# violetdenim/c3dgs

Measured on AMD Instinct MI355X. Metric: raster views/sec fwd+bwd @1920x1080, higher is better.
Workload: dtype f32; 1 GPU; BASELINE.json configs[2]: synth-v1 3M Gaussians, SH deg 3, indexed-camera rasterizer (QAT inner loop), mark_visible+fwd+bwd, 1 view/step/GPU; gaussians=3000000, width=1920, height=1080, sh_codebook=304096, gaussian_codebook=754096, parallelism=replicas x1

## Files before the change

### c3dgs_amd/csrc/radix_sort.hip

```cpp
#include "common.hpp"
#include "scan_blocks.hpp"
#include <algorithm>
#include <cstdlib>
#include <type_traits>

namespace c3dgs {

constexpr int OS_RADIX = 256;
#ifndef C3DGS_OS_TILE32
#define C3DGS_OS_TILE32 12288
#endif
#ifndef C3DGS_OS_BLOCK32
#define C3DGS_OS_BLOCK32 512
#endif
constexpr int OS_TILE16 = 8192, OS_BLOCK16 = 1024;
template <class K> struct OsShape {
    static constexpr int TILE = sizeof(K) == 2 ? OS_TILE16 : C3DGS_OS_TILE32;
    static constexpr int BLOCK = sizeof(K) == 2 ? OS_BLOCK16 : C3DGS_OS_BLOCK32;
    static constexpr int IPT = TILE / BLOCK;
};
constexpr uint32_t OS_FLAG_AGG = 1u << 30, OS_FLAG_PRE = 2u << 30, OS_CNT_MASK = (1u << 30) - 1;
constexpr int OS_MAX_PASSES = 4;
#ifndef C3DGS_OS_SPIN_LIMIT
#define C3DGS_OS_SPIN_LIMIT (1u << 22)
#endif
constexpr uint32_t OS_SPIN_LIMIT = C3DGS_OS_SPIN_LIMIT;
__device__ uint32_t g_os_error;
#ifdef C3DGS_DIAG
__device__ unsigned long long g_os_times[64 * 8];
#endif
#ifdef C3DGS_OS_TIMING
#define OS_T(slot) if (tid == 0 && (bid & 3) == 0 && (bid >> 2) < 64) g_os_times[(bid >> 2) * 8 + (slot)] = __builtin_readcyclecounter();
#define OS_T_DRAIN() asm volatile("s_waitcnt vmcnt(0)");
#define OS_T_LOADS_DONE()                                                                                    \
    if (key[0] == (K)0x12345678 && val[OS_IPT - 1] == 0x87654321u) kout[0] = key[OS_IPT - 1];                \
    OS_T_DRAIN()
#else
#define OS_T(slot)
#define OS_T_DRAIN()
#define OS_T_LOADS_DONE()
#endif

struct OsPlan { int passes; int bits[OS_MAX_PASSES]; };

constexpr int OS_RADIX3 = 512, OS_BITS3 = 9, OS_BITS3_TOP = 32 - 3 * OS_BITS3;
static_assert(OS_RADIX3 == C3DGS_OS_BLOCK32, "one thread per digit in the biased depth sort's passes");
static_assert(OS_RADIX3 == (1 << DEPTH_SORT3_BITS) && 3 * OS_BITS3 == 27 && DEPTH_KEY_LIMIT3 == DEPTH_KEY_BIAS + (1u << 27) - 1u, "common.hpp's plan");
template <bool XF> __device__ __forceinline__ uint32_t os_digit_src(uint32_t k) { return XF ? depth_key_biased(k) : k; }

static OsPlan os_plan(int total_bits)
{
    OsPlan p;
    p.passes = (total_bits + 7) / 8;
    if (p.passes < 1) p.passes = 1;
    int left = total_bits < 1 ? 1 : total_bits;
    for (int i = 0; i < p.passes; i++) {
        const int b = (left + (p.passes - i) - 1) / (p.passes - i);
        p.bits[i] = b;
        left -= b;
    }
    return p;
}

template <class K> static size_t os_blocks(size_t n) { return (n + OsShape<K>::TILE - 1) / OsShape<K>::TILE; }
template <class K> constexpr bool os_table_driven() { return sizeof(K) == 2; }
template <class K> static size_t os_table_words(size_t n) { return os_table_driven<K>() ? os_blocks<K>(n) * OS_RADIX : 0; }
template <class K> static size_t os_lookback_words(size_t n, int passes)
{
    return os_table_driven<K>() ? 0 : (size_t)passes * os_blocks<K>(n) * OS_RADIX + 64;
}
template <class K> static size_t os_ctrl_bytes(size_t n, int passes)
{
    return align_up(((size_t)passes * OS_RADIX + os_lookback_words<K>(n, passes) + os_table_words<K>(n)) * sizeof(uint32_t));
}

constexpr int OS_HIST_BLOCK = 1024;
template <class K>
__device__ __forceinline__ void os_hist_body(const K* __restrict__ keys, size_t n, const OsPlan& plan, uint32_t* __restrict__ hist,
                                             unsigned block, unsigned nblocks)
{
    __shared__ uint32_t s_h[OS_MAX_PASSES][OS_RADIX];
    for (int q = threadIdx.x; q < OS_MAX_PASSES * OS_RADIX; q += OS_HIST_BLOCK) (&s_h[0][0])[q] = 0;
    __syncthreads();
    constexpr int VEC = 16 / sizeof(K);
    const size_t nvec = n / VEC;
    const uint4* k4 = reinterpret_cast<const uint4*>(keys);
    auto add = [&](uint32_t k) {
        int shift = 0;
        for (int p = 0; p < plan.passes; p++) {
            atomicAdd(&s_h[p][(k >> shift) & ((1u << plan.bits[p]) - 1u)], 1u);
            shift += plan.bits[p];
        }
    };
    auto add4 = [&](const uint4 v) {
        const uint32_t w[4] = { v.x, v.y, v.z, v.w };
#pragma unroll
        for (int e = 0; e < 4; e++) {
            if (sizeof(K) == 4) add(w[e]);
            else { add(w[e] & 0xffffu); add(w[e] >> 16); }
        }
    };
    const size_t stride = (size_t)nblocks * OS_HIST_BLOCK;
    size_t i = (size_t)block * OS_HIST_BLOCK + threadIdx.x;
    for (; i + 3 * stride < nvec; i += 4 * stride) {
        const uint4 v0 = k4[i], v1 = k4[i + stride], v2 = k4[i + 2 * stride], v3 = k4[i + 3 * stride];
        add4(v0); add4(v1); add4(v2); add4(v3);
    }
    for (; i < nvec; i += stride) add4(k4[i]);
    for (size_t j = nvec * VEC + (size_t)block * OS_HIST_BLOCK + threadIdx.x; j < n; j += stride) add((uint32_t)keys[j]);
    __syncthreads();
    for (int q = threadIdx.x; q < plan.passes * OS_RADIX; q += OS_HIST_BLOCK) {
        const uint32_t v = (&s_h[0][0])[q];
        if (v) atomicAdd(&hist[q], v);
    }
}

template <class K>
__global__ void __launch_bounds__(OS_HIST_BLOCK) os_hist_kernel(const K* __restrict__ keys, size_t n, OsPlan plan, uint32_t* __restrict__ hist)
{
    os_hist_body<K>(keys, n, plan, hist, blockIdx.x, gridDim.x);
}

static_assert(SCAN_BLOCKS_THREADS == OS_HIST_BLOCK, "one workgroup shape for both bodies");
__global__ void __launch_bounds__(OS_HIST_BLOCK)
os_hist_scan_kernel(const uint32_t* __restrict__ keys, size_t n, OsPlan plan, uint32_t* __restrict__ hist, int nb, uint32_t* __restrict__ base,
                    const uint32_t* __restrict__ sort_err, uint32_t* __restrict__ host_out, uint32_t host_seq)
{
    if (blockIdx.x == 0) scan_blocks_body(nb, base, sort_err, host_out, host_seq);
    else os_hist_body<uint32_t>(keys, n, plan, hist, blockIdx.x - 1, gridDim.x - 1);
}

__device__ __forceinline__ void os_hist3_body(const uint32_t* __restrict__ keys, size_t n, uint32_t* __restrict__ hist, uint32_t* __restrict__ maxw,
                                              uint32_t* __restrict__ done, uint32_t* __restrict__ host_max, uint32_t host_seq,
                                              unsigned block, unsigned nblocks)
{
    __shared__ uint32_t s_h[3][OS_RADIX3];
    __shared__ uint32_t s_max;
    for (int q = threadIdx.x; q < 3 * OS_RADIX3; q += OS_HIST_BLOCK) (&s_h[0][0])[q] = 0;
    if (threadIdx.x == 0) s_max = 0;
    __syncthreads();
    uint32_t mx = 0;
    auto add = [&](uint32_t k) {
        const uint32_t t = depth_key_biased(k);
        atomicAdd(&s_h[0][t & (OS_RADIX3 - 1)], 1u);
        atomicAdd(&s_h[1][(t >> OS_BITS3) & (OS_RADIX3 - 1)], 1u);
        atomicAdd(&s_h[2][(t >> (2 * OS_BITS3)) & (OS_RADIX3 - 1)], 1u);
        if (k != DEPTH_KEY_CULLED) mx = max(mx, k);
    };
    auto add4 = [&](const uint4 v) { add(v.x); add(v.y); add(v.z); add(v.w); };
    const size_t nvec = n / 4;
    const uint4* k4 = reinterpret_cast<const uint4*>(keys);
    const size_t stride = (size_t)nblocks * OS_HIST_BLOCK;
    size_t i = (size_t)block * OS_HIST_BLOCK + threadIdx.x;
    for (; i + 3 * stride < nvec; i += 4 * stride) {
        const uint4 v0 = k4[i], v1 = k4[i + stride], v2 = k4[i + 2 * stride], v3 = k4[i + 3 * stride];
        add4(v0); add4(v1); add4(v2); add4(v3);
    }
    for (; i < nvec; i += stride) add4(k4[i]);
    for (size_t j = nvec * 4 + (size_t)block * OS_HIST_BLOCK + threadIdx.x; j < n; j += stride) add(keys[j]);
#pragma unroll
    for (int o = 32; o > 0; o >>= 1) mx = max(mx, (uint32_t)__shfl_xor((int)mx, o));
    if ((threadIdx.x & 63) == 0 && mx) atomicMax(&s_max, mx);
    __syncthreads();
    for (int q = threadIdx.x; q < 3 * OS_RADIX3; q += OS_HIST_BLOCK) {
        const uint32_t v = (&s_h[0][0])[q];
        if (v) atomicAdd(&hist[q], v);
    }
    if (threadIdx.x == 0) {
        if (s_max) __hip_atomic_fetch_max(maxw, s_max, __ATOMIC_RELAXED, __HIP_MEMORY_SCOPE_AGENT);
        const uint32_t before = __hip_atomic_fetch_add(done, 1u, __ATOMIC_ACQ_REL, __HIP_MEMORY_SCOPE_AGENT);
        if (before == nblocks - 1 && host_max) {
            const uint32_t m = __hip_atomic_load(maxw, __ATOMIC_RELAXED, __HIP_MEMORY_SCOPE_AGENT);
            __hip_atomic_store(host_max, m, __ATOMIC_RELAXED, __HIP_MEMORY_SCOPE_SYSTEM);
            __hip_atomic_store(host_max + 1, host_seq, __ATOMIC_RELEASE, __HIP_MEMORY_SCOPE_SYSTEM);
        }
    }
}

__global__ void __launch_bounds__(OS_HIST_BLOCK)
os_hist3_scan_kernel(const uint32_t* __restrict__ keys, size_t n, uint32_t* __restrict__ hist, uint32_t* __restrict__ maxw, uint32_t* __restrict__ done,
                     uint32_t* __restrict__ host_max, int nb, uint32_t* __restrict__ base, const uint32_t* __restrict__ sort_err,
                     uint32_t* __restrict__ host_out, uint32_t host_seq)
{
    if (blockIdx.x == 0) scan_blocks_body(nb, base, sort_err, host_out, host_seq);
    else os_hist3_body(keys, n, hist, maxw, done, host_max, host_seq, blockIdx.x - 1, gridDim.x - 1);
}

__global__ void __launch_bounds__(OS_HIST_BLOCK) os_hist3_top_kernel(const uint32_t* __restrict__ keys, size_t n, uint32_t* __restrict__ hist)
{
    __shared__ uint32_t s_h[1 << OS_BITS3_TOP];
    if (threadIdx.x < (1 << OS_BITS3_TOP)) s_h[threadIdx.x] = 0;
    __syncthreads();
    const size_t stride = (size_t)gridDim.x * OS_HIST_BLOCK;
    const size_t rounds = (n + stride - 1) / stride;
    for (size_t r = 0; r < rounds; r++) {
        const size_t i = r * stride + (size_t)blockIdx.x * OS_HIST_BLOCK + threadIdx.x;
        const bool ok = i < n;
        const uint32_t d = ok ? depth_key_biased(keys[i]) >> (3 * OS_BITS3) : 0u;
        unsigned long long left = __ballot(ok);
        while (left) {
            const int leader = __ffsll((long long)left) - 1;
            const uint32_t dl = (uint32_t)__shfl((int)d, leader);
            const unsigned long long same = __ballot(ok && d == dl) & left;
            if ((int)(threadIdx.x & 63) == leader) atomicAdd(&s_h[dl], (uint32_t)__popcll(same));
            left &= ~same;
        }
    }
    __syncthreads();
    if (threadIdx.x < (1 << OS_BITS3_TOP) && s_h[threadIdx.x]) atomicAdd(&hist[threadIdx.x], s_h[threadIdx.x]);
}

__global__ void __launch_bounds__(1024) os_tile_hist_kernel(const uint16_t* __restrict__ keys, uint32_t n, int shift, int bits, uint32_t* __restrict__ table)
{
    constexpr int TILE = OsShape<uint16_t>::TILE;
    static_assert(TILE == 8 * 1024, "one 16-byte load of 8 keys per thread");
    __shared__ uint32_t s_h[OS_RADIX];
    if (threadIdx.x < OS_RADIX) s_h[threadIdx.x] = 0;
    __syncthreads();
    const uint32_t base = blockIdx.x * (uint32_t)TILE + threadIdx.x * 8u;
    const uint32_t mask = (1u << bits) - 1u;
    auto add = [&](uint32_t k) { atomicAdd(&s_h[(k >> shift) & mask], 1u); };
    if (base + 8 <= n && (reinterpret_cast<uintptr_t>(keys) & 15u) == 0) {
        const uint4 v = *reinterpret_cast<const uint4*>(keys + base);
        const uint32_t w[4] = { v.x, v.y, v.z, v.w };
#pragma unroll
        for (int e = 0; e < 4; e++) { add(w[e] & 0xffffu); add(w[e] >> 16); }
    } else {
        for (uint32_t i = base; i < min(base + 8u, n); i++) add((uint32_t)keys[i]);
    }
    __syncthreads();
    const int t = threadIdx.x;
    if (t < (1 << bits)) table[(size_t)t * gridDim.x + blockIdx.x] = s_h[t];
}

constexpr int OS_SCAN_V = 8;
__global__ void __launch_bounds__(256) os_table_scan_kernel(uint32_t* __restrict__ table, uint32_t blocks, uint32_t* __restrict__ hist)
{
    static_assert(OS_RADIX == 256, "one thread per histogram word");
    __shared__ uint32_t s_w[4];
    const int digit = (int)blockIdx.x;
    uint32_t* column = table + (size_t)digit * blocks;
    const int lane = threadIdx.x & 63, wave = threadIdx.x >> 6;
    if (digit == 0 && threadIdx.x >= gridDim.x) hist[threadIdx.x] = 0u;
    uint32_t carry = 0;
    for (uint32_t b0 = 0; b0 < blocks; b0 += 256 * OS_SCAN_V) {
        const uint32_t b = b0 + threadIdx.x * OS_SCAN_V;
        uint32_t c[OS_SCAN_V], mine = 0;
#pragma unroll
        for (int q = 0; q < OS_SCAN_V; q++) { c[q] = b + q < blocks ? column[b + q] : 0u; mine += c[q]; }
        uint32_t incl = mine;
#pragma unroll
        for (int o = 1; o < 64; o <<= 1) { const uint32_t t = __shfl_up(incl, o); if (lane >= o) incl += t; }
        __syncthreads();
        if (lane == 63) s_w[wave] = incl;
        __syncthreads();
        uint32_t run = carry + incl - mine;
        for (int w = 0; w < wave; w++) run += s_w[w];
#pragma unroll
        for (int q = 0; q < OS_SCAN_V; q++) { if (b + q < blocks) column[b + q] = run; run += c[q]; }
        carry += s_w[0] + s_w[1] + s_w[2] + s_w[3];
    }
    if (threadIdx.x == 0) hist[digit] = carry;
}

__device__ __forceinline__ uint32_t os_load(const uint32_t* p) { return __hip_atomic_load(p, __ATOMIC_RELAXED, __HIP_MEMORY_SCOPE_AGENT); }
__device__ __forceinline__ void os_store(uint32_t* p, uint32_t v) { __hip_atomic_store(p, v, __ATOMIC_RELAXED, __HIP_MEMORY_SCOPE_AGENT); }

__device__ __forceinline__ uint32_t os_pack_rect(uint2 r)
{
    return (r.x & 0xffu) | ((r.x >> 16) << 8) | ((r.y & 0xffu) << 16) | ((r.y >> 16) << 24);
}
__device__ __forceinline__ uint2 os_unpack_rect(uint32_t w)
{
    return make_uint2((w & 0xffu) | (((w >> 8) & 0xffu) << 16), ((w >> 16) & 0xffu) | ((w >> 24) << 16));
}

template <class K, int BITS, bool PRE, bool PAY2 = false, int RADIX = OS_RADIX, bool XF = false>
__global__ void __launch_bounds__(OsShape<K>::BLOCK)
os_pass_kernel(const K* __restrict__ kin, K* __restrict__ kout, const uint32_t* __restrict__ vin, uint32_t* __restrict__ vout,
               uint32_t n, int shift, const uint32_t* __restrict__ hist, uint32_t* __restrict__ status, uint32_t* __restrict__ ticket,
               const uint2* __restrict__ gather_src, uint2* __restrict__ gather_dst, const uint32_t* __restrict__ p2in = nullptr,
               uint32_t* __restrict__ p2out = nullptr)
{
    constexpr uint32_t ERR_BIT = sizeof(K) == 2 ? 1u : 2u;
    constexpr uint32_t MASK = (1u << BITS) - 1;
    constexpr int OS_BLOCK = OsShape<K>::BLOCK, OS_IPT = OsShape<K>::IPT, OS_WAVES = OS_BLOCK / 64;
    constexpr int OS_TILE = OsShape<K>::TILE;
    using CNT = typename std::conditional<(RADIX > 256), uint16_t, uint32_t>::type;
    static_assert(RADIX % 64 == 0 && RADIX <= OS_BLOCK && BITS <= 9 && (1 << BITS) <= RADIX, "one thread per digit");
    static_assert(!XF || sizeof(K) == 4, "the transform is the depth keys'");
    static_assert(sizeof(CNT) == 4 || OS_TILE < 65536, "a 16-bit counter holds up to a tile's items");
    static_assert(sizeof(CNT) * OS_WAVES * RADIX + 8 * RADIX + 4 * (RADIX / 64) + 4 + sizeof(K) * OS_TILE + 4 * OS_TILE * (PAY2 ? 2 : 1) + (PAY2 ? 0 : 4)
                      <= 160 * 1024, "LDS of one workgroup (160 KB per CU)");
    __shared__ CNT s_cnt[OS_WAVES][RADIX];
    __shared__ uint32_t s_start[RADIX];
    __shared__ int32_t s_gbase[RADIX];
    __shared__ uint32_t s_wtot[RADIX / 64];
    __shared__ uint32_t s_bid;
    __shared__ K s_keys[OS_TILE];
    __shared__ uint32_t s_vals[OS_TILE];
    __shared__ uint32_t s_vals2[PAY2 ? OS_TILE : 1];

    const int tid = threadIdx.x, lane = tid & 63, wave = tid >> 6;
    if (tid == 0) s_bid = PRE ? blockIdx.x : atomicAdd(ticket, 1u);
    for (int q = tid; q < OS_WAVES * RADIX; q += OS_BLOCK) (&s_cnt[0][0])[q] = 0;
    __syncthreads();
    const uint32_t bid = s_bid;
    OS_T(0)
    const uint32_t block_start = bid * (uint32_t)OS_TILE;
    const uint32_t valid = min((uint32_t)OS_TILE, n - block_start);

    K key[OS_IPT];
    uint32_t val[OS_IPT], rank[OS_IPT];
    uint32_t val2[PAY2 ? OS_IPT : 1];
    const uint32_t wbase = block_start + (uint32_t)wave * 64u * OS_IPT;
#pragma unroll
    for (int k = 0; k < OS_IPT; k++) {
        const uint32_t idx = wbase + (uint32_t)k * 64u + lane;
        const bool ok = idx < n;
        key[k] = ok ? kin[idx] : (K)0;
        val[k] = ok ? (vin ? vin[idx] : idx) : 0u;
        if (PAY2) val2[k] = ok ? (p2in ? p2in[idx] : os_pack_rect(gather_src[idx])) : 0u;
    }
    const uint32_t lt_lo = lane < 32 ? (1u << lane) - 1u : 0xffffffffu, lt_hi = lane < 32 ? 0u : (1u << (lane - 32)) - 1u;
    OS_T_LOADS_DONE()
    OS_T(1)
    CNT* wc = s_cnt[wave];
#pragma unroll
    for (int k = 0; k < OS_IPT; k++) {
        const uint32_t idx = wbase + (uint32_t)k * 64u + lane;
        const bool ok = idx < n;
        const uint32_t d = (os_digit_src<XF>((uint32_t)key[k]) >> shift) & MASK;
        const unsigned long long okb = __ballot(ok);
        uint32_t plo = (uint32_t)okb, phi = (uint32_t)(okb >> 32);
#pragma unroll
        for (int b = 0; b < BITS; b++) {
            const int sgn = __builtin_amdgcn_sbfe((int)d, b, 1);
            const unsigned long long bal = __ballot(sgn != 0);
            plo &= ~((uint32_t)bal ^ (uint32_t)sgn);
            phi &= ~((uint32_t)(bal >> 32) ^ (uint32_t)sgn);
        }
        rank[k] = 0;
        if (ok) {
            const uint32_t before = __hip_atomic_load(&wc[d], __ATOMIC_RELAXED, __HIP_MEMORY_SCOPE_WAVEFRONT);
            const uint32_t below = (uint32_t)__popc(plo & lt_lo) + (uint32_t)__popc(phi & lt_hi);
            rank[k] = before + below;
            if (below == 0) __hip_atomic_store(&wc[d], (CNT)(before + (uint32_t)__popc(plo) + (uint32_t)__popc(phi)), __ATOMIC_RELAXED, __HIP_MEMORY_SCOPE_WAVEFRONT);
        }
        __builtin_amdgcn_fence(__ATOMIC_RELEASE, "wavefront");
        __builtin_amdgcn_wave_barrier();
        __builtin_amdgcn_fence(__ATOMIC_ACQUIRE, "wavefront");
    }
    OS_T(2)
    __syncthreads();
    OS_T(3)
    uint32_t tot = 0;
    if (tid < RADIX) {
#pragma unroll
        for (int w = 0; w < OS_WAVES; w++) { const uint32_t c = s_cnt[w][tid]; s_cnt[w][tid] = (CNT)tot; tot += c; }
    }
    uint32_t incl = tot;
#pragma unroll
    for (int o = 1; o < 64; o <<= 1) { const uint32_t t = __shfl_up(incl, o); if (lane >= o) incl += t; }
    if (tid < RADIX && lane == 63) s_wtot[wave] = incl;
    __syncthreads();
    uint32_t start = 0, pre = 0;
    if (tid < RADIX) {
        uint32_t off = 0;
        for (int w = 0; w < wave; w++) off += s_wtot[w];
        start = off + incl - tot;
        s_start[tid] = start;
        uint32_t* my = status + (size_t)bid * RADIX + tid;
        if (PRE) pre = tid < (1 << BITS) ? status[(size_t)tid * gridDim.x + bid] : 0u;
        else if (bid == 0) os_store(my, OS_FLAG_PRE | tot);
        else {
            os_store(my, OS_FLAG_AGG | tot);
            for (int64_t b = (int64_t)bid - 1;; b--) {
                uint32_t s, spins = 0;
                do { s = os_load(status + (size_t)b * RADIX + tid); } while ((s >> 30) == 0 && ++spins < OS_SPIN_LIMIT);
                if ((s >> 30) == 0) { atomicOr(&g_os_error, ERR_BIT); break; }
                pre += s & OS_CNT_MASK;
                if (s & OS_FLAG_PRE) break;
            }
            os_store(my, OS_FLAG_PRE | (pre + tot));
        }
    }
    OS_T(4)
    const uint32_t h = tid < RADIX ? hist[tid] : 0u;
    uint32_t hincl = h;
#pragma unroll
    for (int o = 1; o < 64; o <<= 1) { const uint32_t t = __shfl_up(hincl, o); if (lane >= o) hincl += t; }
    __syncthreads();
    if (tid < RADIX && lane == 63) s_wtot[wave] = hincl;
    __syncthreads();
    if (tid < RADIX) {
        uint32_t off = 0;
        for (int w = 0; w < wave; w++) off += s_wtot[w];
        s_gbase[tid] = (int32_t)(off + hincl - h + pre) - (int32_t)start;
    }
    OS_T(5)
#pragma unroll
    for (int k = 0; k < OS_IPT; k++) {
        const uint32_t idx = wbase + (uint32_t)k * 64u + lane;
        if (idx < n) {
            const uint32_t d = (os_digit_src<XF>((uint32_t)key[k]) >> shift) & MASK;
            const uint32_t p = s_start[d] + s_cnt[wave][d] + rank[k];
            s_keys[p] = key[k];
            s_vals[p] = val[k];
            if (PAY2) s_vals2[p] = val2[k];
        }
    }
    __syncthreads();
    OS_T(6)
#pragma unroll
    for (int m = 0; m < OS_IPT; m++) {
        const uint32_t p = (uint32_t)tid + (uint32_t)m * OS_BLOCK;
        if (p < valid) {
            const K kk = s_keys[p];
            const uint32_t d = (os_digit_src<XF>((uint32_t)kk) >> shift) & MASK;
            const uint32_t g = (uint32_t)(s_gbase[d] + (int32_t)p);
            kout[g] = kk;
            const uint32_t vv = s_vals[p];
            vout[g] = vv;
            if (PAY2) {
                if (p2out) p2out[g] = s_vals2[p];
                else gather_dst[g] = os_unpack_rect(s_vals2[p]);
            } else if (gather_src) gather_dst[g] = gather_src[vv];
        }
    }
    OS_T_DRAIN()
    OS_T(7)
}

template <class K, bool PRE>
static void os_launch_pass(int bits, unsigned blocks, hipStream_t s, const K* ki, K* ko, const uint32_t* vi, uint32_t* vo, uint32_t n,
                           int shift, const uint32_t* hist, uint32_t* status, uint32_t* ticket, const uint2* gsrc, uint2* gdst)
{
#define C3DGS_OS_CASE(B) case B: os_pass_kernel<K, B, PRE><<<blocks, OsShape<K>::BLOCK, 0, s>>>(ki, ko, vi, vo, n, shift, hist, status, ticket, gsrc, gdst); break
    switch (bits) {
        C3DGS_OS_CASE(1); C3DGS_OS_CASE(2); C3DGS_OS_CASE(3); C3DGS_OS_CASE(4);
        C3DGS_OS_CASE(5); C3DGS_OS_CASE(6); C3DGS_OS_CASE(7);
        default: os_pass_kernel<K, 8, PRE><<<blocks, OsShape<K>::BLOCK, 0, s>>>(ki, ko, vi, vo, n, shift, hist, status, ticket, gsrc, gdst); break;
    }
#undef C3DGS_OS_CASE
}

template <class K> static unsigned os_hist_blocks(size_t n)
{
    const size_t nvec16 = n * sizeof(K) / 16 + 1;
    return (unsigned)std::min<size_t>((nvec16 + OS_HIST_BLOCK * 4 - 1) / (OS_HIST_BLOCK * 4), 512);
}

template <class K>
static size_t os_temp_bytes(size_t n, int total_bits, bool pay2 = false)
{
    const OsPlan plan = os_plan(total_bits);
    size_t b = os_ctrl_bytes<K>(n, plan.passes);
    const int bufs = plan.passes >= 3 ? 2 : (plan.passes == 2 ? 1 : 0);
    b += (size_t)bufs * (align_up(n * sizeof(K)) + align_up(n * sizeof(uint32_t)));
    if (pay2) b += 2 * align_up(n * sizeof(uint32_t));
    return b;
}

template <class K>
static size_t os_clear_bytes(size_t n, int total_bits)
{
    if (os_table_driven<K>()) return 0;
    return os_ctrl_bytes<K>(n, os_plan(total_bits).passes);
}

template <class K>
static hipError_t os_sort(void* temp, size_t temp_bytes, const K* kin, K* kout, const uint32_t* vin, uint32_t* vout, size_t n,
                          int total_bits, hipStream_t s, const uint2* gather_src = nullptr, uint2* gather_dst = nullptr,
                          bool ctrl_cleared = false, bool pay2 = false, bool hist_done = false)
{
    if (n == 0) return hipSuccess;
    if (pay2 && (sizeof(K) != 4 || total_bits != 32 || !gather_src || !gather_dst || vin || os_temp_bytes<K>(n, total_bits, true) > temp_bytes))
        pay2 = false;
    if (n >= ((size_t)1 << 30) || total_bits > 8 * (int)sizeof(K) || os_temp_bytes<K>(n, total_bits) > temp_bytes) return hipErrorInvalidValue;
    const OsPlan plan = os_plan(total_bits);
    const size_t blocks = os_blocks<K>(n);
    char* base = (char*)temp;
    const size_t ctrl = os_ctrl_bytes<K>(n, plan.passes);
    uint32_t* hist = (uint32_t*)base;
    uint32_t* behind_hist = hist + (size_t)plan.passes * OS_RADIX;
    K* tk[2]; uint32_t* tv[2];
    char* q = base + ctrl;
    for (int i = 0; i < 2; i++) { tk[i] = (K*)q; q += align_up(n * sizeof(K)); tv[i] = (uint32_t*)q; q += align_up(n * sizeof(uint32_t)); }
    if constexpr (os_table_driven<K>()) {
        uint32_t* table = behind_hist;
        int shift = 0;
        for (int p = 0; p < plan.passes; p++) {
            const bool last = p == plan.passes - 1;
            const K* ki = p == 0 ? kin : tk[(p - 1) & 1];
            const uint32_t* vi = p == 0 ? vin : tv[(p - 1) & 1];
            uint32_t* h = hist + (size_t)p * OS_RADIX;
            os_tile_hist_kernel<<<(unsigned)blocks, 1024, 0, s>>>((const uint16_t*)ki, (uint32_t)n, shift, plan.bits[p], table);
            os_table_scan_kernel<<<1u << plan.bits[p], 256, 0, s>>>(table, (uint32_t)blocks, h);
            os_launch_pass<K, true>(plan.bits[p], (unsigned)blocks, s, ki, last ? kout : tk[p & 1], vi, last ? vout : tv[p & 1], (uint32_t)n,
                                    shift, h, table, nullptr, last ? gather_src : nullptr, last ? gather_dst : nullptr);
            shift += plan.bits[p];
        }
        return hipGetLastError();
    } else {
        uint32_t* status = behind_hist;
        uint32_t* ticket = status + (size_t)plan.passes * blocks * OS_RADIX;
        uint32_t* t2[2] = { nullptr, nullptr };
        if (pay2) {
            q = base + os_temp_bytes<K>(n, total_bits);
            for (int i = 0; i < 2; i++) { t2[i] = (uint32_t*)q; q += align_up(n * sizeof(uint32_t)); }
        }
        if (!ctrl_cleared) {
            const hipError_t e = hipMemsetAsync(base, 0, os_clear_bytes<K>(n, total_bits), s);
            if (e != hipSuccess) return e;
        }
        if (!hist_done) os_hist_kernel<K><<<os_hist_blocks<K>(n), OS_HIST_BLOCK, 0, s>>>(kin, n, plan, hist);
        int shift = 0;
        for (int p = 0; p < plan.passes; p++) {
            const K* ki = p == 0 ? kin : tk[(p - 1) & 1];
            const uint32_t* vi = p == 0 ? vin : tv[(p - 1) & 1];
            K* ko = p == plan.passes - 1 ? kout : tk[p & 1];
            uint32_t* vo = p == plan.passes - 1 ? vout : tv[p & 1];
            const bool last = p == plan.passes - 1;
            if (pay2)
                os_pass_kernel<K, 8, false, true><<<(unsigned)blocks, OsShape<K>::BLOCK, 0, s>>>(
                    ki, ko, vi, vo, (uint32_t)n, shift, hist + (size_t)p * OS_RADIX, status + (size_t)p * blocks * OS_RADIX, ticket + p,
                    gather_src, gather_dst, p == 0 ? nullptr : t2[(p - 1) & 1], last ? nullptr : t2[p & 1]);
            else
                os_launch_pass<K, false>(plan.bits[p], (unsigned)blocks, s, ki, ko, vi, vo, (uint32_t)n, shift, hist + (size_t)p * OS_RADIX,
                                         status + (size_t)p * blocks * OS_RADIX, ticket + p, last ? gather_src : nullptr, last ? gather_dst : nullptr);
            shift += plan.bits[p];
        }
        return hipGetLastError();
    }
}

struct Os3Layout {
    size_t blocks, ctrl_bytes, total_bytes;
    uint32_t *hist[4], *status[4], *ticket, *maxw, *done;
    uint32_t *tk[2], *tv[2], *t2[2];
};
static Os3Layout os3_layout(void* temp, size_t n)
{
    Os3Layout L;
    L.blocks = os_blocks<uint32_t>(n);
    const size_t hist_words = 3 * OS_RADIX3 + OS_RADIX, status_words = L.blocks * hist_words;
    L.ctrl_bytes = align_up((hist_words + status_words + 64) * sizeof(uint32_t));
    uint32_t* w = (uint32_t*)temp;
    for (int p = 0; p < 4; p++) {
        L.hist[p] = w + (size_t)p * OS_RADIX3;
        L.status[p] = w + hist_words + (size_t)p * L.blocks * OS_RADIX3;
    }
    L.ticket = w + hist_words + status_words;
    L.maxw = L.ticket + 8;
    L.done = L.ticket + 9;
    char* q = (char*)temp + L.ctrl_bytes;
    const size_t a = align_up(n * sizeof(uint32_t));
    for (int i = 0; i < 2; i++) { L.tk[i] = (uint32_t*)q; q += a; L.tv[i] = (uint32_t*)q; q += a; }
    for (int i = 0; i < 2; i++) { L.t2[i] = (uint32_t*)q; q += a; }
    L.total_bytes = (size_t)(q - (char*)temp);
    return L;
}
static bool os3_args_ok(size_t temp_bytes, int P)
{
    return P > 0 && (size_t)P < ((size_t)1 << 30) && os3_layout(nullptr, (size_t)P).total_bytes <= temp_bytes;
}

hipError_t onesweep_depth3_hist_scan(void* temp, size_t temp_bytes, const uint32_t* keys, int P, int nb, uint32_t* base,
                                     const uint32_t* sort_err, uint32_t* host_out, uint32_t host_seq, uint32_t* host_max, hipStream_t s)
{
    if (!os3_args_ok(temp_bytes, P)) return hipErrorInvalidValue;
    const Os3Layout L = os3_layout(temp, (size_t)P);
    os_hist3_scan_kernel<<<1u + os_hist_blocks<uint32_t>((size_t)P), OS_HIST_BLOCK, 0, s>>>(keys, (size_t)P, L.hist[0], L.maxw, L.done, host_max, nb,
                                                                                            base, sort_err, host_out, host_seq);
    return hipGetLastError();
}
const uint32_t* onesweep_depth3_max_word(void* temp, int P) { return os3_layout(temp, (size_t)(P > 0 ? P : 1)).maxw; }

hipError_t onesweep_depth3_head(void* temp, size_t temp_bytes, const uint32_t* kin, int P, const uint2* rects, hipStream_t s)
{
    if (!os3_args_ok(temp_bytes, P) || !rects) return hipErrorInvalidValue;
    const Os3Layout L = os3_layout(temp, (size_t)P);
    const unsigned blocks = (unsigned)L.blocks;
    os_pass_kernel<uint32_t, OS_BITS3, false, true, OS_RADIX3, true><<<blocks, C3DGS_OS_BLOCK32, 0, s>>>(
        kin, L.tk[0], nullptr, L.tv[0], (uint32_t)P, 0, L.hist[0], L.status[0], L.ticket + 0, rects, nullptr, nullptr, L.t2[0]);
    os_pass_kernel<uint32_t, OS_BITS3, false, true, OS_RADIX3, true><<<blocks, C3DGS_OS_BLOCK32, 0, s>>>(
        L.tk[0], L.tk[1], L.tv[0], L.tv[1], (uint32_t)P, OS_BITS3, L.hist[1], L.status[1], L.ticket + 1, rects, nullptr, L.t2[0], L.t2[1]);
    return hipGetLastError();
}
hipError_t onesweep_depth3_tail(void* temp, size_t temp_bytes, const uint32_t* kin, uint32_t* kout, uint32_t* vout, int P,
                                const uint2* rects, uint2* rects_sorted, uint32_t max_visible_key, hipStream_t s)
{
    if (!os3_args_ok(temp_bytes, P) || !rects || !rects_sorted) return hipErrorInvalidValue;
    const Os3Layout L = os3_layout(temp, (size_t)P);
    const unsigned blocks = (unsigned)L.blocks;
    const bool four = depth_sort_plan(true, max_visible_key).passes == 4;
    os_pass_kernel<uint32_t, OS_BITS3, false, true, OS_RADIX3, true><<<blocks, C3DGS_OS_BLOCK32, 0, s>>>(
        L.tk[1], four ? L.tk[0] : kout, L.tv[1], four ? L.tv[0] : vout, (uint32_t)P, 2 * OS_BITS3, L.hist[2], L.status[2], L.ticket + 2, rects,
        rects_sorted, L.t2[1], four ? L.t2[0] : nullptr);
    if (four) {
        os_hist3_top_kernel<<<os_hist_blocks<uint32_t>((size_t)P), OS_HIST_BLOCK, 0, s>>>(kin, (size_t)P, L.hist[3]);
        os_pass_kernel<uint32_t, OS_BITS3_TOP, false, true, OS_RADIX, true><<<blocks, C3DGS_OS_BLOCK32, 0, s>>>(
            L.tk[0], kout, L.tv[0], vout, (uint32_t)P, 3 * OS_BITS3, L.hist[3], L.status[3], L.ticket + 3, rects, rects_sorted, L.t2[0], nullptr);
    }
    return hipGetLastError();
}

#ifdef C3DGS_DIAG
int os_read_times(unsigned long long* out512)
{
    return hipMemcpyFromSymbol(out512, HIP_SYMBOL(g_os_times), sizeof(unsigned long long) * 512) != hipSuccess;
}
#endif

uint32_t* onesweep_error_word()
{
    static uint32_t* cache[64] = { nullptr };
    int dev = 0;
    if (hipGetDevice(&dev) != hipSuccess || dev < 0 || dev >= 64) return nullptr;
    if (!cache[dev]) {
        void* p = nullptr;
        if (hipGetSymbolAddress(&p, HIP_SYMBOL(g_os_error)) != hipSuccess) return nullptr;
        cache[dev] = (uint32_t*)p;
    }
    return cache[dev];
}

int onesweep_timed_out(hipStream_t s)
{
    if (!onesweep_enabled()) return 0;
    uint32_t* e = onesweep_error_word();
    uint32_t w = 1;
    if (!e || hipMemcpyAsync(&w, e, sizeof(w), hipMemcpyDeviceToHost, s) != hipSuccess) return 1;
    if (hipStreamSynchronize(s) != hipSuccess) return 1;
    if (w) (void)hipMemsetAsync(e, 0, sizeof(w), s);
    return w != 0;
}

bool onesweep_enabled()
{
    static const bool on = []() { const char* e = std::getenv("C3DGS_SORT_ROCPRIM"); return !(e && e[0] == '1'); }();
    return on;
}
size_t onesweep_depth_temp_bytes(int P)
{
    const size_t n = (size_t)(P > 0 ? P : 1);
    return std::max(os_temp_bytes<uint32_t>(n, 32, true), os3_layout(nullptr, n).total_bytes);
}
size_t onesweep_tile_temp_bytes(int R, int end_bit, int key_bytes)
{
    return key_bytes == 4 ? os_temp_bytes<uint32_t>((size_t)(R > 0 ? R : 1), end_bit) : os_temp_bytes<uint16_t>((size_t)(R > 0 ? R : 1), end_bit);
}
size_t onesweep_depth_clear_bytes(int P)
{
    const size_t n = (size_t)(P > 0 ? P : 1);
    return std::max(os_clear_bytes<uint32_t>(n, 32), os3_layout(nullptr, n).ctrl_bytes);
}
size_t onesweep_tile_clear_bytes(int R, int end_bit, int key_bytes)
{
    return key_bytes == 4 ? os_clear_bytes<uint32_t>((size_t)(R > 0 ? R : 1), end_bit) : os_clear_bytes<uint16_t>((size_t)(R > 0 ? R : 1), end_bit);
}
hipError_t onesweep_tile_sort32(void* temp, size_t temp_bytes, const uint32_t* kin, uint32_t* kout, const uint32_t* vin, uint32_t* vout,
                                int R, int end_bit, hipStream_t s, bool ctrl_cleared)
{
    return os_sort<uint32_t>(temp, temp_bytes, kin, kout, vin, vout, (size_t)R, end_bit, s, nullptr, nullptr, ctrl_cleared);
}
hipError_t onesweep_depth_hist_scan(void* temp, size_t temp_bytes, const uint32_t* keys, int P, int nb, uint32_t* base,
                                    const uint32_t* sort_err, uint32_t* host_out, uint32_t host_seq, hipStream_t s)
{
    const size_t n = (size_t)P;
    if (P <= 0 || n >= ((size_t)1 << 30) || os_temp_bytes<uint32_t>(n, 32) > temp_bytes) return hipErrorInvalidValue;
    os_hist_scan_kernel<<<1u + os_hist_blocks<uint32_t>(n), OS_HIST_BLOCK, 0, s>>>(keys, n, os_plan(32), (uint32_t*)temp, nb, base,
                                                                                  sort_err, host_out, host_seq);
    return hipGetLastError();
}
hipError_t onesweep_depth_sort(void* temp, size_t temp_bytes, const uint32_t* kin, uint32_t* kout, const uint32_t* vin, uint32_t* vout,
                               int P, const uint2* gather_src, uint2* gather_dst, hipStream_t s, bool ctrl_cleared, bool rects_fit_bytes,
                               bool hist_done)
{
    static const bool no_pay2 = []() { const char* e = std::getenv("C3DGS_DEPTH_SORT_GATHER"); return e && e[0] == '1'; }();
    return os_sort<uint32_t>(temp, temp_bytes, kin, kout, vin, vout, (size_t)P, 32, s, gather_src, gather_dst, ctrl_cleared,
                             rects_fit_bytes && !no_pay2, hist_done && ctrl_cleared);
}
hipError_t onesweep_tile_sort(void* temp, size_t temp_bytes, const uint16_t* kin, uint16_t* kout, const uint32_t* vin, uint32_t* vout,
                              int R, int end_bit, hipStream_t s, bool ctrl_cleared)
{
    return os_sort<uint16_t>(temp, temp_bytes, kin, kout, vin, vout, (size_t)R, end_bit, s, nullptr, nullptr, ctrl_cleared);
}

}
```

Before: 646.9 views/s.

## Carry only the high digit byte between u16 radix passes and rebuild keys

In the table-driven 16-bit key sort, the first pass now writes only the upper-digit byte to a uint8 plane instead of full u16 keys. The second pass reads that byte plane and rebuilds the low digit from the bucket start offsets of the first pass (a scan of the first histogram done in the second hist kernel), using a binary search over the bucket starts. This halves intermediate key traffic and temp memory. It adds a binary search per thread plus extra kernel template variants, and the scheme assumes at most two passes.

```diff
diff --git a/c3dgs_amd/csrc/radix_sort.hip b/c3dgs_amd/csrc/radix_sort.hip
--- a/c3dgs_amd/csrc/radix_sort.hip
+++ b/c3dgs_amd/csrc/radix_sort.hip
@@ -65,13 +65,14 @@
 template <class K> static size_t os_blocks(size_t n) { return (n + OsShape<K>::TILE - 1) / OsShape<K>::TILE; }
 template <class K> constexpr bool os_table_driven() { return sizeof(K) == 2; }
 template <class K> static size_t os_table_words(size_t n) { return os_table_driven<K>() ? os_blocks<K>(n) * OS_RADIX : 0; }
+template <class K> constexpr size_t os_lo_words() { return os_table_driven<K>() ? OS_RADIX + 8 : 0; }
 template <class K> static size_t os_lookback_words(size_t n, int passes)
 {
     return os_table_driven<K>() ? 0 : (size_t)passes * os_blocks<K>(n) * OS_RADIX + 64;
 }
 template <class K> static size_t os_ctrl_bytes(size_t n, int passes)
 {
-    return align_up(((size_t)passes * OS_RADIX + os_lookback_words<K>(n, passes) + os_table_words<K>(n)) * sizeof(uint32_t));
+    return align_up(((size_t)passes * OS_RADIX + os_lookback_words<K>(n, passes) + os_lo_words<K>() + os_table_words<K>(n)) * sizeof(uint32_t));
 }
 
 constexpr int OS_HIST_BLOCK = 1024;
@@ -210,10 +211,12 @@
     if (threadIdx.x < (1 << OS_BITS3_TOP) && s_h[threadIdx.x]) atomicAdd(&hist[threadIdx.x], s_h[threadIdx.x]);
 }
 
-__global__ void __launch_bounds__(1024) os_tile_hist_kernel(const uint16_t* __restrict__ keys, uint32_t n, int shift, int bits, uint32_t* __restrict__ table)
+template <class K>
+__global__ void __launch_bounds__(1024) os_tile_hist_kernel(const K* __restrict__ keys, uint32_t n, int shift, int bits, uint32_t* __restrict__ table,
+                                                            const uint32_t* __restrict__ lo_hist = nullptr, uint32_t* __restrict__ lo_start = nullptr)
 {
     constexpr int TILE = OsShape<uint16_t>::TILE;
-    static_assert(TILE == 8 * 1024, "one 16-byte load of 8 keys per thread");
+    static_assert(TILE == 8 * 1024 && (sizeof(K) == 1 || sizeof(K) == 2), "one load of 8 keys per thread: 16 bytes of u16, 8 of u8");
     __shared__ uint32_t s_h[OS_RADIX];
     if (threadIdx.x < OS_RADIX) s_h[threadIdx.x] = 0;
     __syncthreads();
@@ -221,16 +224,41 @@
     const uint32_t mask = (1u << bits) - 1u;
     auto add = [&](uint32_t k) { atomicAdd(&s_h[(k >> shift) & mask], 1u); };
     if (base + 8 <= n && (reinterpret_cast<uintptr_t>(keys) & 15u) == 0) {
-        const uint4 v = *reinterpret_cast<const uint4*>(keys + base);
-        const uint32_t w[4] = { v.x, v.y, v.z, v.w };
-#pragma unroll
-        for (int e = 0; e < 4; e++) { add(w[e] & 0xffffu); add(w[e] >> 16); }
+        if constexpr (sizeof(K) == 2) {
+            const uint4 v = *reinterpret_cast<const uint4*>(keys + base);
+            const uint32_t w[4] = { v.x, v.y, v.z, v.w };
+#pragma unroll
+            for (int e = 0; e < 4; e++) { add(w[e] & 0xffffu); add(w[e] >> 16); }
+        } else {
+            const uint2 v = *reinterpret_cast<const uint2*>(keys + base);
+            const uint32_t w[2] = { v.x, v.y };
+#pragma unroll
+            for (int e = 0; e < 2; e++) { add(w[e] & 0xffu); add((w[e] >> 8) & 0xffu); add((w[e] >> 16) & 0xffu); add(w[e] >> 24); }
+        }
     } else {
         for (uint32_t i = base; i < min(base + 8u, n); i++) add((uint32_t)keys[i]);
     }
     __syncthreads();
     const int t = threadIdx.x;
     if (t < (1 << bits)) table[(size_t)t * gridDim.x + blockIdx.x] = s_h[t];
+    if constexpr (sizeof(K) == 1) {
+        if (blockIdx.x == 0 && lo_start) {
+            __shared__ uint32_t s_w[OS_RADIX / 64];
+            const int lane = t & 63, wave = t >> 6;
+            const uint32_t h = t < OS_RADIX ? lo_hist[t] : 0u;
+            uint32_t incl = h;
+#pragma unroll
+            for (int o = 1; o < 64; o <<= 1) { const uint32_t v = __shfl_up(incl, o); if (lane >= o) incl += v; }
+            if (t < OS_RADIX && lane == 63) s_w[wave] = incl;
+            __syncthreads();
+            if (t < OS_RADIX) {
+                uint32_t off = 0;
+                for (int w = 0; w < wave; w++) off += s_w[w];
+                lo_start[t] = off + incl - h;
+            }
+            if (t == 0) lo_start[OS_RADIX] = n;
+        }
+    }
 }
 
 constexpr int OS_SCAN_V = 8;
@@ -275,13 +303,16 @@
     return make_uint2((w & 0xffu) | (((w >> 8) & 0xffu) << 16), ((w >> 16) & 0xffu) | ((w >> 24) << 16));
 }
 
-template <class K, int BITS, bool PRE, bool PAY2 = false, int RADIX = OS_RADIX, bool XF = false>
+constexpr int OS_PLANE_NONE = 0, OS_PLANE_WRITE = 1, OS_PLANE_READ = 2;
+template <class K, int BITS, bool PRE, bool PAY2 = false, int RADIX = OS_RADIX, bool XF = false, int PLANE = OS_PLANE_NONE>
 __global__ void __launch_bounds__(OsShape<K>::BLOCK)
 os_pass_kernel(const K* __restrict__ kin, K* __restrict__ kout, const uint32_t* __restrict__ vin, uint32_t* __restrict__ vout,
                uint32_t n, int shift, const uint32_t* __restrict__ hist, uint32_t* __restrict__ status, uint32_t* __restrict__ ticket,
                const uint2* __restrict__ gather_src, uint2* __restrict__ gather_dst, const uint32_t* __restrict__ p2in = nullptr,
-               uint32_t* __restrict__ p2out = nullptr)
-{
+               uint32_t* __restrict__ p2out = nullptr, const uint8_t* __restrict__ plane_in = nullptr, uint8_t* __restrict__ plane_out = nullptr,
+               const uint32_t* __restrict__ lo_start = nullptr)
+{
+    static_assert(PLANE == OS_PLANE_NONE || (sizeof(K) == 2 && PRE && !PAY2 && !XF && RADIX == OS_RADIX), "the digit plane is the table-driven u16 sort's");
     constexpr uint32_t ERR_BIT = sizeof(K) == 2 ? 1u : 2u;
     constexpr uint32_t MASK = (1u << BITS) - 1;
     constexpr int OS_BLOCK = OsShape<K>::BLOCK, OS_IPT = OsShape<K>::IPT, OS_WAVES = OS_BLOCK / 64;
@@ -291,7 +322,7 @@
     static_assert(!XF || sizeof(K) == 4, "the transform is the depth keys'");
     static_assert(sizeof(CNT) == 4 || OS_TILE < 65536, "a 16-bit counter holds up to a tile's items");
     static_assert(sizeof(CNT) * OS_WAVES * RADIX + 8 * RADIX + 4 * (RADIX / 64) + 4 + sizeof(K) * OS_TILE + 4 * OS_TILE * (PAY2 ? 2 : 1) + (PAY2 ? 0 : 4)
-                      <= 160 * 1024, "LDS of one workgroup (160 KB per CU)");
+                      + 4 * (PLANE == OS_PLANE_READ ? RADIX + 1 : 1) <= 160 * 1024, "LDS of one workgroup (160 KB per CU)");
     __shared__ CNT s_cnt[OS_WAVES][RADIX];
     __shared__ uint32_t s_start[RADIX];
     __shared__ int32_t s_gbase[RADIX];
@@ -300,10 +331,13 @@
     __shared__ K s_keys[OS_TILE];
     __shared__ uint32_t s_vals[OS_TILE];
     __shared__ uint32_t s_vals2[PAY2 ? OS_TILE : 1];
+    __shared__ uint32_t s_lo[PLANE == OS_PLANE_READ ? RADIX + 1 : 1];
 
     const int tid = threadIdx.x, lane = tid & 63, wave = tid >> 6;
     if (tid == 0) s_bid = PRE ? blockIdx.x : atomicAdd(ticket, 1u);
     for (int q = tid; q < OS_WAVES * RADIX; q += OS_BLOCK) (&s_cnt[0][0])[q] = 0;
+    uint32_t lo_v = 0;
+    if constexpr (PLANE == OS_PLANE_READ) { if (tid <= RADIX) lo_v = lo_start[tid]; }
     __syncthreads();
     const uint32_t bid = s_bid;
     OS_T(0)
@@ -318,7 +352,8 @@
     for (int k = 0; k < OS_IPT; k++) {
         const uint32_t idx = wbase + (uint32_t)k * 64u + lane;
         const bool ok = idx < n;
-        key[k] = ok ? kin[idx] : (K)0;
+        if constexpr (PLANE == OS_PLANE_READ) key[k] = ok ? (K)plane_in[idx] : (K)0;
+        else key[k] = ok ? kin[idx] : (K)0;
         val[k] = ok ? (vin ? vin[idx] : idx) : 0u;
         if (PAY2) val2[k] = ok ? (p2in ? p2in[idx] : os_pack_rect(gather_src[idx])) : 0u;
     }
@@ -330,7 +365,7 @@
     for (int k = 0; k < OS_IPT; k++) {
         const uint32_t idx = wbase + (uint32_t)k * 64u + lane;
         const bool ok = idx < n;
-        const uint32_t d = (os_digit_src<XF>((uint32_t)key[k]) >> shift) & MASK;
+        const uint32_t d = PLANE == OS_PLANE_READ ? (uint32_t)key[k] & MASK : (os_digit_src<XF>((uint32_t)key[k]) >> shift) & MASK;
         const unsigned long long okb = __ballot(ok);
         uint32_t plo = (uint32_t)okb, phi = (uint32_t)(okb >> 32);
 #pragma unroll
@@ -352,8 +387,26 @@
         __builtin_amdgcn_fence(__ATOMIC_ACQUIRE, "wavefront");
     }
     OS_T(2)
+    if constexpr (PLANE == OS_PLANE_READ) { if (tid <= RADIX) s_lo[tid] = lo_v; }
     __syncthreads();
     OS_T(3)
+    if constexpr (PLANE == OS_PLANE_READ) {
+        if (wbase + lane < n) {
+            uint32_t lo_d = 0;
+#pragma unroll
+            for (int step = RADIX / 2; step > 0; step >>= 1)
+                if (s_lo[lo_d + step] <= wbase + lane) lo_d += step;
+            uint32_t lo_next = s_lo[lo_d + 1];
+#pragma unroll
+            for (int k = 0; k < OS_IPT; k++) {
+                const uint32_t idx = wbase + (uint32_t)k * 64u + lane;
+                if (idx < n) {
+                    while (idx >= lo_next) lo_next = s_lo[++lo_d + 1];
+                    key[k] = (K)(((uint32_t)key[k] << shift) | lo_d);
+                }
+            }
+        }
+    }
     uint32_t tot = 0;
     if (tid < RADIX) {
 #pragma unroll
@@ -419,7 +472,8 @@
             const K kk = s_keys[p];
             const uint32_t d = (os_digit_src<XF>((uint32_t)kk) >> shift) & MASK;
             const uint32_t g = (uint32_t)(s_gbase[d] + (int32_t)p);
-            kout[g] = kk;
+            if constexpr (PLANE == OS_PLANE_WRITE) plane_out[g] = (uint8_t)((uint32_t)kk >> (shift + BITS));
+            else kout[g] = kk;
             const uint32_t vv = s_vals[p];
             vout[g] = vv;
             if (PAY2) {
@@ -445,6 +499,23 @@
 #undef C3DGS_OS_CASE
 }
 
+static void os_launch_plane_write(int bits, unsigned blocks, hipStream_t s, const uint16_t* ki, uint8_t* plane, const uint32_t* vi, uint32_t* ids,
+                                  uint32_t n, const uint32_t* hist, uint32_t* table)
+{
+#define C3DGS_OS_CASE(B) case B: os_pass_kernel<uint16_t, B, true, false, OS_RADIX, false, OS_PLANE_WRITE><<<blocks, OS_BLOCK16, 0, s>>>( \
+        ki, nullptr, vi, ids, n, 0, hist, table, nullptr, nullptr, nullptr, nullptr, nullptr, nullptr, plane, nullptr); break
+    switch (bits) { C3DGS_OS_CASE(5); C3DGS_OS_CASE(6); C3DGS_OS_CASE(7); default: C3DGS_OS_CASE(8); }
+#undef C3DGS_OS_CASE
+}
+static void os_launch_plane_read(int bits, unsigned blocks, hipStream_t s, const uint8_t* plane, uint16_t* ko, const uint32_t* ids, uint32_t* vo,
+                                 uint32_t n, int shift, const uint32_t* hist, uint32_t* table, const uint32_t* lo_start)
+{
+#define C3DGS_OS_CASE(B) case B: os_pass_kernel<uint16_t, B, true, false, OS_RADIX, false, OS_PLANE_READ><<<blocks, OS_BLOCK16, 0, s>>>( \
+        nullptr, ko, ids, vo, n, shift, hist, table, nullptr, nullptr, nullptr, nullptr, nullptr, plane, nullptr, lo_start); break
+    switch (bits) { C3DGS_OS_CASE(4); C3DGS_OS_CASE(5); C3DGS_OS_CASE(6); C3DGS_OS_CASE(7); default: C3DGS_OS_CASE(8); }
+#undef C3DGS_OS_CASE
+}
+
 template <class K> static unsigned os_hist_blocks(size_t n)
 {
     const size_t nvec16 = n * sizeof(K) / 16 + 1;
@@ -457,7 +528,8 @@
     const OsPlan plan = os_plan(total_bits);
     size_t b = os_ctrl_bytes<K>(n, plan.passes);
     const int bufs = plan.passes >= 3 ? 2 : (plan.passes == 2 ? 1 : 0);
-    b += (size_t)bufs * (align_up(n * sizeof(K)) + align_up(n * sizeof(uint32_t)));
+    const size_t between = os_table_driven<K>() ? sizeof(uint8_t) : sizeof(K);
+    b += (size_t)bufs * (align_up(n * between) + align_up(n * sizeof(uint32_t)));
     if (pay2) b += 2 * align_up(n * sizeof(uint32_t));
     return b;
 }
@@ -488,19 +560,20 @@
     char* q = base + ctrl;
     for (int i = 0; i < 2; i++) { tk[i] = (K*)q; q += align_up(n * sizeof(K)); tv[i] = (uint32_t*)q; q += align_up(n * sizeof(uint32_t)); }
     if constexpr (os_table_driven<K>()) {
-        uint32_t* table = behind_hist;
-        int shift = 0;
-        for (int p = 0; p < plan.passes; p++) {
-            const bool last = p == plan.passes - 1;
-            const K* ki = p == 0 ? kin : tk[(p - 1) & 1];
-            const uint32_t* vi = p == 0 ? vin : tv[(p - 1) & 1];
-            uint32_t* h = hist + (size_t)p * OS_RADIX;
-            os_tile_hist_kernel<<<(unsigned)blocks, 1024, 0, s>>>((const uint16_t*)ki, (uint32_t)n, shift, plan.bits[p], table);
-            os_table_scan_kernel<<<1u << plan.bits[p], 256, 0, s>>>(table, (uint32_t)blocks, h);
-            os_launch_pass<K, true>(plan.bits[p], (unsigned)blocks, s, ki, last ? kout : tk[p & 1], vi, last ? vout : tv[p & 1], (uint32_t)n,
-                                    shift, h, table, nullptr, last ? gather_src : nullptr, last ? gather_dst : nullptr);
-            shift += plan.bits[p];
-        }
+        uint32_t* lo_start = behind_hist;
+        uint32_t* table = behind_hist + os_lo_words<K>();
+        os_tile_hist_kernel<uint16_t><<<(unsigned)blocks, 1024, 0, s>>>((const uint16_t*)kin, (uint32_t)n, 0, plan.bits[0], table);
+        os_table_scan_kernel<<<1u << plan.bits[0], 256, 0, s>>>(table, (uint32_t)blocks, hist);
+        if (plan.passes == 1) {
+            os_launch_pass<K, true>(plan.bits[0], (unsigned)blocks, s, kin, kout, vin, vout, (uint32_t)n, 0, hist, table, nullptr, gather_src, gather_dst);
+            return hipGetLastError();
+        }
+        uint8_t* plane = (uint8_t*)(base + ctrl);
+        uint32_t* ids = (uint32_t*)(base + ctrl + align_up(n * sizeof(uint8_t)));
+        os_launch_plane_write(plan.bits[0], (unsigned)blocks, s, (const uint16_t*)kin, plane, vin, ids, (uint32_t)n, hist, table);
+        os_tile_hist_kernel<uint8_t><<<(unsigned)blocks, 1024, 0, s>>>(plane, (uint32_t)n, 0, plan.bits[1], table, hist, lo_start);
+        os_table_scan_kernel<<<1u << plan.bits[1], 256, 0, s>>>(table, (uint32_t)blocks, hist + OS_RADIX);
+        os_launch_plane_read(plan.bits[1], (unsigned)blocks, s, plane, (uint16_t*)kout, ids, vout, (uint32_t)n, plan.bits[0], hist + OS_RADIX, table, lo_start);
         return hipGetLastError();
     } else {
         uint32_t* status = behind_hist;
```

Result: no change. 646.7 views/s (-0.0%).
